# 10XGenomics/rust-pseudoaligner

Hardware: AMD Instinct MI355X
Metric: reads/sec pseudoaligned (whole node) on synthetic 150bp reads (higher is better)
Workload: dtype u64; 1 GPU; config3: ~202k-transcript synthetic GENCODE-scale index (K=24), error-free 150bp reads; read_len=150, k=24, transcripts=201914, kmers=103866252, index_bytes=7185579820

## Files before the change

### rust-pseudoaligner_amd/csrc/count_sort.hip

```cpp
#include <hip/hip_runtime.h>

#include <algorithm>

#include "kernels.hpp"
#include "pa_common.hpp"

namespace pa {
namespace {

constexpr uint32_t NO_KEY = 0xFFFFFFFFu;
#ifndef PA_MAX_BINS
#define PA_MAX_BINS 256
#endif
constexpr uint32_t MAX_BINS = PA_MAX_BINS;
constexpr uint64_t PA_COUNT_DIRECT_MAX_READS = 1u << 16;
constexpr uint32_t BIN_SLOTS = 1u << PA_KEY_BIN_SHIFT;
constexpr uint32_t CS_BLOCK = 1024;

struct KeyTops {
    const unsigned long long* top;
    uint64_t cap;
    const unsigned long long* extra_top;
    uint64_t extra_cap;
};
__device__ __forceinline__ uint64_t stream_len(const KeyTops k, uint64_t unused = 0) {
    (void)unused;
    unsigned long long t = *k.top, x = k.extra_top ? *k.extra_top : 0ull;
    if (t > k.cap) t = k.cap;
    if (x > k.extra_cap) x = k.extra_cap;
    return t + x;
}

constexpr uint32_t PT_BLOCK = 512, PT_PER = 16, PT_TILE = PT_BLOCK * PT_PER;

__device__ __forceinline__ uint64_t main_len(const KeyTops k) { const unsigned long long t = *k.top; return t < k.cap ? t : k.cap; }
__device__ __forceinline__ uint64_t extra_len(const KeyTops k) {
    const unsigned long long x = k.extra_top ? *k.extra_top : 0ull;
    return x < k.extra_cap ? x : k.extra_cap;
}
__device__ __forceinline__ uint32_t tiles_of(uint64_t n) { return (uint32_t)((n + PT_TILE - 1) / PT_TILE); }

__global__ __launch_bounds__(PT_BLOCK) void pa_keys_part_kernel(const uint32_t* __restrict__ keys, const KeyTops keys_top, uint32_t pass, uint32_t nbins,
                                                                uint32_t tcap, uint16_t* __restrict__ sorted, uint32_t* __restrict__ run_off) {
    __shared__ uint32_t cnt[MAX_BINS], lbase[MAX_BINS + 1];
    __shared__ __attribute__((aligned(16))) uint16_t stage[PT_TILE];
    const uint64_t m = main_len(keys_top);
    const uint64_t seg0 = pass ? m : 0, len = pass ? extra_len(keys_top) : m;
    const uint32_t tile0 = pass ? tiles_of(m) : 0u, ntiles = tiles_of(len);
    for (uint32_t t = blockIdx.x; t < ntiles; t += gridDim.x) {
        for (uint32_t b = threadIdx.x; b < nbins; b += PT_BLOCK) cnt[b] = 0;
        __syncthreads();
        const uint64_t t0 = (uint64_t)t * PT_TILE;
        uint32_t k[PT_PER], pos[PT_PER];
        const uint4* src = reinterpret_cast<const uint4*>(keys + seg0 + t0) + threadIdx.x;
#pragma unroll
        for (uint32_t j = 0; j < PT_PER / 4; ++j) {
            const uint64_t i = t0 + 4ull * (j * PT_BLOCK + threadIdx.x);
            const uint4 v = i < len ? src[j * PT_BLOCK] : uint4{NO_KEY, NO_KEY, NO_KEY, NO_KEY};
            k[4 * j] = v.x; k[4 * j + 1] = v.y; k[4 * j + 2] = v.z; k[4 * j + 3] = v.w;
        }
#pragma unroll
        for (uint32_t j = 0; j < PT_PER; ++j) pos[j] = k[j] != NO_KEY ? atomicAdd(&cnt[k[j] >> PA_KEY_BIN_SHIFT], 1u) : 0u;
        __syncthreads();
        for (uint32_t b = threadIdx.x; b <= nbins; b += PT_BLOCK) {
            uint32_t s = 0;
            for (uint32_t j = 0; j < b; ++j) s += cnt[j];
            lbase[b] = s;
            run_off[(uint64_t)b * tcap + tile0 + t] = s;
        }
        __syncthreads();
#pragma unroll
        for (uint32_t j = 0; j < PT_PER; ++j)
            if (k[j] != NO_KEY) stage[lbase[k[j] >> PA_KEY_BIN_SHIFT] + pos[j]] = (uint16_t)(k[j] & (BIN_SLOTS - 1));
        __syncthreads();
        uint4* dst = reinterpret_cast<uint4*>(sorted + (uint64_t)(tile0 + t) * PT_TILE);
        const uint32_t n8 = (lbase[nbins] + 7) / 8;
        for (uint32_t i = threadIdx.x; i < n8; i += PT_BLOCK) dst[i] = reinterpret_cast<const uint4*>(stage)[i];
        __syncthreads();
    }
}

constexpr uint32_t CG_LANES = 16, CG_DEPTH = 8;
__global__ __launch_bounds__(CS_BLOCK) void pa_keys_count_kernel(const uint16_t* __restrict__ src, const uint32_t* __restrict__ run_off, uint32_t tcap,
                                                                 const KeyTops keys_top, uint32_t parts, unsigned long long* __restrict__ counts,
                                                                 uint64_t counts_len) {
    extern __shared__ uint32_t tab[];
    const uint32_t bin = blockIdx.x / parts, part = blockIdx.x % parts;
    const uint64_t slot0 = (uint64_t)bin << PA_KEY_BIN_SHIFT;
    const uint32_t nslots = (uint32_t)(counts_len - slot0 < BIN_SLOTS ? counts_len - slot0 : BIN_SLOTS);
    for (uint32_t i = threadIdx.x; i < nslots; i += CS_BLOCK) tab[i] = 0;
    __syncthreads();
    const uint32_t ntiles = tiles_of(main_len(keys_top)) + tiles_of(extra_len(keys_top));
    const uint32_t ta = (uint32_t)((uint64_t)ntiles * part / parts), tb = (uint32_t)((uint64_t)ntiles * (part + 1) / parts);
    const uint32_t gl = threadIdx.x % CG_LANES, group = threadIdx.x / CG_LANES;
    const uint4* q = reinterpret_cast<const uint4*>(src);
    for (uint32_t t = ta + group; t < tb; t += CS_BLOCK / CG_LANES) {
        const uint64_t base = (uint64_t)t * PT_TILE;
        const uint64_t a = base + run_off[(uint64_t)bin * tcap + t], b = base + run_off[(uint64_t)(bin + 1) * tcap + t];
        const uint64_t a8 = (a + 7) & ~7ull, b8 = b & ~7ull;
        if (a8 >= b8) {
            for (uint64_t i = a + gl; i < b; i += CG_LANES) atomicAdd(&tab[src[i]], 1u);
            continue;
        }
        const uint32_t head = a + gl < a8 ? src[a + gl] : 0xFFFFu, tail = b8 + gl < b ? src[b8 + gl] : 0xFFFFu;
        for (uint64_t o0 = a8 / 8; o0 < b8 / 8; o0 += (uint64_t)CG_DEPTH * CG_LANES) {
            uint4 v[CG_DEPTH];
            bool in[CG_DEPTH];
#pragma unroll
            for (uint32_t j = 0; j < CG_DEPTH; ++j) {
                const uint64_t o = o0 + (uint64_t)j * CG_LANES + gl;
                in[j] = o < b8 / 8;
                v[j] = in[j] ? q[o] : uint4{0u, 0u, 0u, 0u};
            }
#pragma unroll
            for (uint32_t j = 0; j < CG_DEPTH; ++j)
                if (in[j]) {
                    atomicAdd(&tab[v[j].x & 0xFFFFu], 1u); atomicAdd(&tab[v[j].x >> 16], 1u);
                    atomicAdd(&tab[v[j].y & 0xFFFFu], 1u); atomicAdd(&tab[v[j].y >> 16], 1u);
                    atomicAdd(&tab[v[j].z & 0xFFFFu], 1u); atomicAdd(&tab[v[j].z >> 16], 1u);
                    atomicAdd(&tab[v[j].w & 0xFFFFu], 1u); atomicAdd(&tab[v[j].w >> 16], 1u);
                }
        }
        if (head != 0xFFFFu) atomicAdd(&tab[head], 1u);
        if (tail != 0xFFFFu) atomicAdd(&tab[tail], 1u);
    }
    __syncthreads();
    for (uint32_t i = threadIdx.x; i < nslots; i += CS_BLOCK) {
        const uint32_t c = tab[i];
        if (c) atomicAdd(counts + slot0 + i, (unsigned long long)c);
    }
}

__global__ __launch_bounds__(CS_BLOCK) void pa_keys_count_raw_kernel(const uint32_t* __restrict__ src, const KeyTops keys_top, unsigned long long* __restrict__ counts,
                                                                     uint64_t counts_len) {
    extern __shared__ uint32_t tab[];
    for (uint32_t i = threadIdx.x; i < counts_len; i += CS_BLOCK) tab[i] = 0;
    __syncthreads();
    const uint64_t n4 = stream_len(keys_top) / 4;
    const uint64_t a = n4 * blockIdx.x / gridDim.x, b = n4 * (blockIdx.x + 1) / gridDim.x;
    const uint4* q = reinterpret_cast<const uint4*>(src);
    for (uint64_t i = a + threadIdx.x; i < b; i += CS_BLOCK) {
        const uint4 v = q[i];
        if (v.x != NO_KEY) atomicAdd(&tab[v.x], 1u);
        if (v.y != NO_KEY) atomicAdd(&tab[v.y], 1u);
        if (v.z != NO_KEY) atomicAdd(&tab[v.z], 1u);
        if (v.w != NO_KEY) atomicAdd(&tab[v.w], 1u);
    }
    __syncthreads();
    for (uint32_t i = threadIdx.x; i < counts_len; i += CS_BLOCK) {
        const uint32_t c = tab[i];
        if (c) atomicAdd(counts + i, (unsigned long long)c);
    }
}

__global__ __launch_bounds__(256) void pa_keys_count_direct_kernel(const uint32_t* __restrict__ keys, const KeyTops keys_top, unsigned long long* __restrict__ counts) {
    const uint64_t n = stream_len(keys_top);
    for (uint64_t i = (uint64_t)blockIdx.x * blockDim.x + threadIdx.x; i < n; i += (uint64_t)gridDim.x * blockDim.x) {
        const uint32_t k = keys[i];
        if (k != NO_KEY) atomicAdd(counts + k, 1ull);
    }
}


}
uint64_t key_stream_capacity(uint64_t n_reads, uint32_t nwaves) {
    return (n_reads / PA_KEY_CHUNK + nwaves + 2) * PA_KEY_CHUNK;
}

static uint64_t nbins_of(uint64_t counts_len) { return (counts_len + BIN_SLOTS - 1) >> PA_KEY_BIN_SHIFT; }

static bool count_direct(uint64_t nbins, uint64_t n_reads) { return nbins > MAX_BINS || (nbins > 1 && n_reads <= PA_COUNT_DIRECT_MAX_READS); }

bool count_keys_partitioned(uint64_t counts_len, uint64_t n_reads) {
    const uint64_t nbins = nbins_of(counts_len);
    return nbins > 1 && !count_direct(nbins, n_reads);
}

static uint32_t tile_capacity(uint64_t keys_cap, uint64_t extra_cap) {
    return (uint32_t)((keys_cap + PT_TILE - 1) / PT_TILE + (extra_cap + PT_TILE - 1) / PT_TILE);
}

void count_keys_scratch(uint64_t counts_len, uint64_t n_reads, uint64_t keys_cap, uint64_t extra_cap, size_t* sorted_bytes, size_t* ctl_bytes) {
    *sorted_bytes = *ctl_bytes = 0;
    if (!count_keys_partitioned(counts_len, n_reads)) return;
    const uint64_t tcap = tile_capacity(keys_cap, extra_cap);
    *sorted_bytes = tcap * PT_TILE * sizeof(uint16_t);
    *ctl_bytes = (nbins_of(counts_len) + 1) * tcap * sizeof(uint32_t);
}

int launch_count_keys(const uint32_t* keys, const unsigned long long* keys_top_ptr, uint64_t keys_cap, const unsigned long long* extra_top, uint64_t extra_cap,
                      uint32_t* sorted, uint32_t* ctl, unsigned long long* counts, uint64_t counts_len, int num_cus, hipStream_t stream, uint64_t n_reads,
                      uint32_t pass) {
    if (counts_len == 0) return 0;
    const KeyTops keys_top{keys_top_ptr, keys_cap, extra_top, extra_cap};
    const uint64_t nbins = nbins_of(counts_len);
    const uint32_t cus = num_cus > 0 ? (uint32_t)num_cus : 256u;
    const bool partitioned = count_keys_partitioned(counts_len, n_reads);
    if (pass == 0) {
        if (!partitioned) return 0;
        const uint32_t tcap = tile_capacity(keys_cap, extra_cap);
        const uint32_t G = std::max<uint32_t>(1u, std::min<uint32_t>(cus * 4, (uint32_t)((keys_cap + PT_TILE - 1) / PT_TILE)));
        hipLaunchKernelGGL(pa_keys_part_kernel, dim3(G), dim3(PT_BLOCK), 0, stream, keys, keys_top, 0u, (uint32_t)nbins, tcap, reinterpret_cast<uint16_t*>(sorted), ctl);
        return (int)hipGetLastError();
    }
    const size_t lds = (size_t)(counts_len < BIN_SLOTS ? counts_len : BIN_SLOTS) * 4;
    if (lds > 48 * 1024) {
        hipError_t e = hipFuncSetAttribute(reinterpret_cast<const void*>(&pa_keys_count_kernel), hipFuncAttributeMaxDynamicSharedMemorySize, (int)lds);
        if (e == hipSuccess) e = hipFuncSetAttribute(reinterpret_cast<const void*>(&pa_keys_count_raw_kernel), hipFuncAttributeMaxDynamicSharedMemorySize, (int)lds);
        if (e != hipSuccess) return (int)e;
    }
    if (count_direct(nbins, n_reads)) {
        const uint32_t blocks = (uint32_t)std::min<uint64_t>((uint64_t)cus * 8, (keys_cap + extra_cap + 255) / 256 + 1);
        hipLaunchKernelGGL(pa_keys_count_direct_kernel, dim3(blocks), dim3(256), 0, stream, keys, keys_top, counts);
        return (int)hipGetLastError();
    }
    if (nbins == 1) {
        hipLaunchKernelGGL(pa_keys_count_raw_kernel, dim3(cus), dim3(CS_BLOCK), lds, stream, keys, keys_top, counts, counts_len);
        return (int)hipGetLastError();
    }
    const uint32_t tcap = tile_capacity(keys_cap, extra_cap);
    const uint32_t G1 = std::max<uint32_t>(1u, std::min<uint32_t>(cus * 4, (uint32_t)((extra_cap + PT_TILE - 1) / PT_TILE)));
    hipLaunchKernelGGL(pa_keys_part_kernel, dim3(G1), dim3(PT_BLOCK), 0, stream, keys, keys_top, 1u, (uint32_t)nbins, tcap, reinterpret_cast<uint16_t*>(sorted), ctl);
    uint32_t parts = std::max<uint32_t>(1u, (uint32_t)(cus / nbins));
    parts = std::max<uint32_t>(1u, (uint32_t)knob_int("PA_COUNT_PARTS", (int)parts));
    hipLaunchKernelGGL(pa_keys_count_kernel, dim3((uint32_t)nbins * parts), dim3(CS_BLOCK), lds, stream, reinterpret_cast<const uint16_t*>(sorted), (const uint32_t*)ctl, tcap,
                       keys_top, parts, counts, counts_len);
    return (int)hipGetLastError();
}

}
```

### rust-pseudoaligner_amd/csrc/device_index.hip

```cpp
#include <hip/hip_runtime.h>

#include <algorithm>
#include <cstdlib>
#include <cstring>
#include <thread>

#include "device_flatten.hpp"
#include "device_index.hpp"
#include "lane_steps.hpp"

using namespace pa;

namespace {

uint64_t list_hash_host(const uint32_t* v, uint32_t n) {
    uint64_t h = 0x243f6a8885a308d3ull ^ n;
    for (uint32_t i = 0; i < n; ++i) h = mix64(h ^ v[i]) + 0x9e3779b97f4a7c15ull;
    return h;
}

}

namespace pa {

void LaunchCtx::release() {
    if (side) (void)hipStreamSynchronize(side);
    ctl.release();
    for (DeviceBuffer<uint32_t>* b : {&spill, &trace, &novel, &keys, &keys_sorted, &keys_ctl, &defer}) b->release();
    for (hipEvent_t e : {ev0, ev1, ev2, ev3, fork, join})
        if (e) (void)hipEventDestroy(e);
    ev0 = ev1 = ev2 = ev3 = fork = join = nullptr;
    if (side) (void)hipStreamDestroy(side);
    side = nullptr;
    timed = false;
}

void* Parked::take(std::mutex& mu) {
    std::lock_guard<std::mutex> g(mu);
    if (held.empty()) return nullptr;
    void* obj = held.back().first;
    held.pop_back();
    return obj;
}
void Parked::put(std::mutex& mu, void* obj, void (*free_fn)(void*)) {
    {
        std::lock_guard<std::mutex> g(mu);
        if (held.size() < cap) {
            held.emplace_back(obj, free_fn);
            return;
        }
    }
    free_fn(obj);
}

void index_host_classes(const pa_index* idx, const uint32_t** ec, const uint32_t** class_ref, int* device) {
    *ec = idx->h_ec.data();
    *class_ref = idx->h_class_ref.data();
    *device = idx->device;
}
void index_pair_view(pa_index* idx, PairIndexView* out) {
    std::lock_guard<std::mutex> g(idx->mu);
    *out = PairIndexView{idx->dv, idx->d_class_table.get(), idx->class_table_size, idx->ovf, idx->device, idx->num_cus};
}
void index_host_class_text(pa_index* idx, const uint64_t** off, const char** text) {
    std::call_once(idx->class_text_once, [idx] {
        const uint32_t nc = idx->stats.num_classes;
        const uint32_t* ec = idx->h_ec.data();
        const uint32_t* cref = idx->h_class_ref.data();
        auto digits = [](uint32_t v) { uint32_t d = 1; while (v >= 10) { v /= 10; ++d; } return d; };
        std::vector<uint64_t>& off_v = idx->h_class_text_off;
        off_v.assign((size_t)nc + 1, 0);
        const int T = std::max(1, std::min(16, usable_threads()));
        const uint32_t* clen = idx->h_class_len.data();
        auto ids_of = [&](uint32_t c, const uint32_t*& ids, uint32_t& n) {
            ids = ec + 4ull * cref[c] + 1;
            n = clen[c];
        };
        {
            std::vector<std::thread> th;
            for (int t = 0; t < T; ++t)
                th.emplace_back([&, t] {
                    for (uint64_t c = (uint64_t)nc * t / T; c < (uint64_t)nc * (t + 1) / T; ++c) {
                        const uint32_t* ids; uint32_t n;
                        ids_of((uint32_t)c, ids, n);
                        uint64_t len = n ? 2ull * (n - 1) : 0;
                        for (uint32_t j = 0; j < n; ++j) len += digits(ids[j]);
                        off_v[c + 1] = len;
                    }
                });
            for (auto& x : th) x.join();
        }
        for (uint32_t c = 0; c < nc; ++c) off_v[c + 1] += off_v[c];
        idx->h_class_text.resize(off_v[nc] + 16);
        {
            std::vector<std::thread> th;
            for (int t = 0; t < T; ++t)
                th.emplace_back([&, t] {
                    for (uint64_t c = (uint64_t)nc * t / T; c < (uint64_t)nc * (t + 1) / T; ++c) {
                        const uint32_t* ids; uint32_t n;
                        ids_of((uint32_t)c, ids, n);
                        char* o = idx->h_class_text.data() + off_v[c];
                        for (uint32_t j = 0; j < n; ++j) {
                            if (j) { *o++ = ','; *o++ = ' '; }
                            char b[10]; int k = 10; uint32_t v = ids[j];
                            do { b[--k] = (char)('0' + v % 10); v /= 10; } while (v);
                            memcpy(o, b + k, (size_t)(10 - k)); o += 10 - k;
                        }
                    }
                });
            for (auto& x : th) x.join();
        }
    });
    *off = idx->h_class_text_off.data();
    *text = idx->h_class_text.data();
}
int index_device_class_text(pa_index* idx, const uint64_t** d_off, const uint8_t** d_text) {
    const uint64_t* off = nullptr;
    const char* txt = nullptr;
    index_host_class_text(idx, &off, &txt);
    std::lock_guard<std::mutex> g(idx->mu);
    if (!idx->d_class_text.get()) {
        if (hipSetDevice(idx->device) != hipSuccess) return fail(PA_ERR_HIP, "hipSetDevice failed");
        int e = upload(idx->d_class_text_off, off, idx->h_class_text_off.size());
        if (e == PA_OK) e = upload(idx->d_class_text, reinterpret_cast<const uint8_t*>(txt), idx->h_class_text.size());
        if (e != PA_OK) return e;
    }
    *d_off = idx->d_class_text_off.get();
    *d_text = idx->d_class_text.get();
    return PA_OK;
}
void* index_take_ingest_cache(pa_index* idx) { return idx->ingest_caches.take(idx->mu); }
void index_put_ingest_cache(pa_index* idx, void* cache, void (*free_fn)(void*)) { idx->ingest_caches.put(idx->mu, cache, free_fn); }
void* index_take_host_pipe(pa_index* idx) { return idx->host_pipes.take(idx->mu); }
void index_put_host_pipe(pa_index* idx, void* pipe, void (*free_fn)(void*)) { idx->host_pipes.put(idx->mu, pipe, free_fn); }

}

extern "C" {

void pa_index_destroy(pa_index* idx) {
    if (!idx) return;
    (void)hipSetDevice(idx->device);
    {
        std::vector<std::pair<void*, void (*)(void*)>> parked;
        { std::lock_guard<std::mutex> g(idx->mu); parked.swap(idx->ingest_caches.held); parked.insert(parked.end(), idx->host_pipes.held.begin(), idx->host_pipes.held.end()); idx->host_pipes.held.clear(); }
        for (auto& c : parked) c.second(c.first);
    }
    for (auto& kv : idx->ctxs) kv.second->release();
    delete idx;
}

int pa_index_create(const pa_flat_index* flat, int device, pa_index** out) {
    if (!flat || !out) return fail(PA_ERR_INVALID_ARG, "null argument");
    int rc = use_device(device);
    if (rc != PA_OK) return rc;
    FlatDevice fd;
    int threads = usable_threads();
    if (threads < 1) threads = 1;
    rc = flatten_for_device(*flat, threads, fd, true);
    if (rc != PA_OK) return rc;

    std::vector<uint32_t> ctab((size_t)fd.num_classes * 2 + 16, 0xFFFFFFFFu);
    for (uint32_t c = 0; c < fd.num_classes; ++c) {
        uint64_t j = list_hash_host(fd.ec.data() + 4ull * fd.class_ref[c] + 1, fd.class_len[c]) % ctab.size();
        while (ctab[j] != 0xFFFFFFFFu)
            if (++j == ctab.size()) j = 0;
        ctab[j] = c;
    }

    pa_index* idx = new (std::nothrow) pa_index();
    if (!idx) return fail(PA_ERR_OOM, "out of memory");
    idx->device = device;
    hipDeviceProp_t prop;
    if (hipGetDeviceProperties(&prop, device) == hipSuccess) idx->num_cus = prop.multiProcessorCount;
    if (idx->num_cus <= 0) idx->num_cus = 256;
    rc = upload(idx->d_blobs, fd.blobs);
    if (rc == PA_OK) rc = upload(idx->d_ledge, fd.ledge);
    if (rc == PA_OK) rc = device_fill_index(fd, idx->d_blobs.get(), idx->d_table, &fd.nbuckets);
    if (rc == PA_OK) rc = upload(idx->d_seg_g, fd.seg_g);
    if (rc == PA_OK) rc = upload(idx->d_seg_nid, fd.seg_nid);
    if (rc == PA_OK) rc = upload(idx->d_ec, fd.ec);
    if (rc == PA_OK) rc = upload(idx->d_class_ref, fd.class_ref);
    if (rc == PA_OK) rc = upload(idx->d_class_len, fd.class_len);
    if (rc == PA_OK) rc = upload(idx->d_class_table, ctab);
    if (rc == PA_OK) rc = upload(idx->d_wtable, fd.wtable);
    if (rc != PA_OK) { pa_index_destroy(idx); return rc; }
    idx->class_table_size = ctab.size();
    idx->dv = fd.host_view();
    idx->dv.table = idx->d_table.get();
    idx->dv.blobs = idx->d_blobs.get();
    idx->dv.ledge = idx->d_ledge.get();
    idx->dv.seg_g = idx->d_seg_g.get();
    idx->dv.seg_nid = idx->d_seg_nid.get();
    idx->h_ec = fd.ec;
    idx->h_class_ref = fd.class_ref;
    idx->h_class_len = fd.class_len;
    idx->dv.ec = idx->d_ec.get();
    idx->dv.class_ref = idx->d_class_ref.get();
    idx->dv.class_len = idx->d_class_len.get();
    idx->dv.wtable = idx->d_wtable.get();
    idx->dv.stream_nt = (fd.k <= 32 && fd.nbuckets * BUCKET_WORDS * 4 > (512ull << 20)) ? 1u : 0u;
    pa_index_stats& s = idx->stats;
    s.num_kmers = fd.num_kmers;
    s.table_slots = fd.nbuckets * SLOTS_PER_BUCKET;
    s.bytes_table = fd.nbuckets * BUCKET_WORDS * 4;
    s.bytes_graph = fd.blobs.size() + fd.ledge.size() * 4 + fd.seg_g.size() * 12;
    s.bytes_classes = (fd.ec.size() + fd.class_ref.size() + fd.class_len.size() + ctab.size() + fd.wtable.size()) * 4;
    s.bytes_total = s.bytes_table + s.bytes_graph + s.bytes_classes;
    s.num_nodes = fd.num_nodes;
    s.num_classes = fd.num_classes;
    s.k = fd.k;
    s.max_class_len = fd.max_class_len;
    *out = idx;
    return PA_OK;
}

int pa_index_create_multi(const pa_flat_index* flat, const int* devices, int ndev, pa_index** out) {
    if (!flat || !devices || !out || ndev < 1) return fail(PA_ERR_INVALID_ARG, "null argument or ndev < 1");
    for (int i = 0; i < ndev; ++i) out[i] = nullptr;
    for (int i = 0; i < ndev; ++i) {
        for (int j = 0; j < i; ++j)
            if (devices[j] == devices[i]) {
                for (int t = 0; t < i; ++t) { pa_index_destroy(out[t]); out[t] = nullptr; }
                return fail(PA_ERR_INVALID_ARG, "device %d listed twice", devices[i]);
            }
        const int rc = pa_index_create(flat, devices[i], &out[i]);
        if (rc != PA_OK) {
            const std::string why = last_error_ref();
            for (int t = 0; t <= i; ++t) { pa_index_destroy(out[t]); out[t] = nullptr; }
            return fail(rc, "device %d: %s", devices[i], why.c_str());
        }
    }
    return PA_OK;
}

int pa_index_get_stats(const pa_index* idx, pa_index_stats* stats) {
    if (!idx || !stats) return fail(PA_ERR_INVALID_ARG, "null argument");
    *stats = idx->stats;
    return PA_OK;
}

uint32_t pa_words_per_read(uint32_t max_read_len) { return (max_read_len + 31) / 32 ? (max_read_len + 31) / 32 : 1; }
size_t pa_tiles_words(uint64_t n_reads, uint32_t words_per_read) { return (size_t)((n_reads + 63) / 64) * words_per_read * 64; }

int pa_encode_reads_device(const pa_index* idx, const uint8_t* d_ascii, const uint64_t* d_offsets, uint64_t n_reads,
                           uint32_t words_per_read, uint64_t* d_tiles, uint32_t* d_lens, void* stream) {
    if (!idx || !d_ascii || !d_offsets || !d_tiles || !d_lens || words_per_read == 0) return fail(PA_ERR_INVALID_ARG, "null argument");
    PA_HIP_TRY(hipSetDevice(idx->device));
    const int e = launch_encode(d_ascii, d_offsets, n_reads, words_per_read, d_tiles, d_lens, static_cast<hipStream_t>(stream));
    if (e) return fail(PA_ERR_HIP, "encode launch: %s", hipGetErrorString((hipError_t)e));
    return PA_OK;
}

}

namespace pa {

static int env_int(const char* name, int dflt) { return knob_int(name, dflt); }

uint32_t spill_cap_of(uint32_t wpr) { return 256 * wpr + 24; }

static int pool_geometry(pa_index* idx, uint64_t n_reads, uint32_t wpr, uint32_t* grid, size_t* lds, uint32_t* slots) {
    const size_t cu_lds = 160 * 1024 - 4096;
    int per_cu = env_int("PA_MAP_BLOCKS_PER_CU", 3);
    uint32_t S = 0;
    for (; per_cu >= 1; --per_cu) {
        const size_t per_wave = cu_lds / (size_t)per_cu / (PA_MAP_BLOCK / 64);
        const size_t per_slot = pool_slot_bytes(wpr);
        if (per_wave < pool_fixed_bytes() + 64 * per_slot + 16) continue;
        S = (uint32_t)((per_wave - pool_fixed_bytes() - 16) / per_slot);
        break;
    }
    if (S < 64) return fail(PA_ERR_UNSUPPORTED, "reads of %u words do not fit the LDS of a compute unit", wpr);
    if (S > pool_max_slots()) S = pool_max_slots();
    const int want = env_int("PA_POOL_SLOTS", 0);
    if (want >= 64 && (uint32_t)want <= S) S = (uint32_t)want;
    *slots = S;
    *lds = pool_lds_bytes(wpr, S);
    int occ = 0;
    if (pool_kernel_occupancy(*lds, &occ) == 0 && occ >= 1 && occ < per_cu) per_cu = occ;
    const uint64_t ntiles = (n_reads + 63) / 64;
    const uint64_t waves_wanted = (ntiles + 7) / 8;
    uint64_t blocks = (waves_wanted + PA_MAP_BLOCK / 64 - 1) / (PA_MAP_BLOCK / 64);
    const uint64_t cap = (uint64_t)idx->num_cus * per_cu;
    if (blocks > cap) blocks = cap;
    if (blocks < 1) blocks = 1;
    *grid = (uint32_t)blocks;
    return PA_OK;
}

static int ctx_of(pa_index* idx, hipStream_t stream, std::shared_ptr<LaunchCtx>* out) {
    std::lock_guard<std::mutex> g(idx->mu);
    auto it = idx->ctxs.find(stream);
    if (it == idx->ctxs.end()) {
        std::shared_ptr<LaunchCtx> c(new (std::nothrow) LaunchCtx());
        if (!c) return fail(PA_ERR_OOM, "out of memory");
        const int rc = grow(c->ctl, 2);
        if (rc != PA_OK) return rc;
        it = idx->ctxs.emplace(stream, std::move(c)).first;
    }
    *out = it->second;
    return PA_OK;
}

int StreamCtx::open(pa_index* idx, hipStream_t stream) {
    PA_HIP_TRY(hipSetDevice(idx->device));
    const int rc = ctx_of(idx, stream, &cx);
    if (rc != PA_OK) return rc;
    lock = std::unique_lock<std::mutex>(cx->mu);
    return PA_OK;
}

int map_launch_locked(pa_index* idx, LaunchCtx* cx, hipStream_t stream, const MapLaunch& m) {
    const uint64_t n_reads = m.n_reads;
    const uint32_t wpr = m.wpr;
    MapCtl* const ctl = cx->ctl.get();
    if (n_reads >= 0xFFFFFFFFull) return fail(PA_ERR_UNSUPPORTED, "at most 2^32-2 reads per batch");
    if (wpr == 0 || wpr > (PA_MAX_READ_LEN + 31) / 32) return fail(PA_ERR_UNSUPPORTED, "words_per_read %u outside [1,%u]", wpr, (PA_MAX_READ_LEN + 31) / 32);
    uint32_t grid = 0;
    size_t lds = 0;
    uint32_t slots = 64;
    int rc = pool_geometry(idx, n_reads, wpr, &grid, &lds, &slots);
    if (rc != PA_OK) return rc;
    const uint32_t spill_cap = spill_cap_of(wpr);
    {
        const size_t per_block = (size_t)(PA_MAP_BLOCK / 64) * slots * spill_cap * 4 * (m.nodes ? 2 : 1);
        const size_t budget = (size_t)6 << 30;
        if ((size_t)grid * per_block > budget) grid = (uint32_t)std::max<size_t>(1, budget / per_block);
    }
    const size_t lanes = (size_t)grid * (PA_MAP_BLOCK / 64) * slots;
    rc = grow(cx->spill, lanes * spill_cap);
    if (rc != PA_OK) return rc;
    if (m.nodes) { rc = grow(cx->trace, lanes * spill_cap); if (rc != PA_OK) return rc; }
    PA_HIP_TRY(hipMemsetAsync(ctl, 0, sizeof(MapCtl), stream));
    MapParams p{};
    p.ix = idx->dv;
    p.tiles = m.tiles;
    p.lens = m.lens;
    p.uniform_len = m.uniform_len;
    p.n_reads = n_reads;
    p.wpr = wpr;
    p.allowed = m.allowed;
    p.results = m.results;
    p.arena = m.arena;
    p.arena_cap = m.arena_cap > PA_MAX_ARENA_ENTRIES ? PA_MAX_ARENA_ENTRIES : m.arena_cap;
    p.colour_out = m.colour;
    p.arena_top = &ctl->arena_top;
    p.status = &ctl->status;
    p.tile_ctr = &ctl->tile_ctr;
    p.spill = cx->spill.get();
    p.spill_cap = spill_cap;
    const uint64_t counts_len = (uint64_t)idx->stats.num_classes + 3;
    const uint64_t defer_cap = defer_capacity(n_reads, grid * (PA_MAP_BLOCK / 64));
    if ((rc = grow(cx->defer, defer_cap * 8))) return rc;
    p.defer = cx->defer.get();
    p.defer_top = &ctl->defer_top;
    p.defer_cap = defer_cap;
    p.keys_cap = 0;
    uint64_t keys_cap = 0;
    if (m.counts) {
        keys_cap = key_stream_capacity(n_reads, grid * (PA_MAP_BLOCK / 64));
        size_t sorted_bytes = 0, ctl_bytes = 0;
        count_keys_scratch(counts_len, n_reads, keys_cap, defer_cap, &sorted_bytes, &ctl_bytes);
        if ((rc = grow(cx->keys, keys_cap + defer_cap)) || (rc = grow(cx->keys_sorted, (sorted_bytes + 3) / 4)) || (rc = grow(cx->keys_ctl, (ctl_bytes + 3) / 4))) return rc;
        p.keys = cx->keys.get();
        p.keys_top = &ctl->keys_top;
        p.keys_cap = keys_cap;
        p.counts = reinterpret_cast<unsigned long long*>(m.counts);
    }
    p.class_table = idx->d_class_table.get();
    p.class_table_size = idx->class_table_size;
    p.pool_slots = slots;
    p.dbg = env_int("PA_MAP_STATS", 0) ? ctl->stats : nullptr;
    p.ablate = (uint32_t)env_int("PA_MAP_ABLATE", 0);
    pa_overflow* ovf = nullptr;
    { std::lock_guard<std::mutex> g(idx->mu); ovf = idx->ovf; }
    if (m.counts && ovf) {
        const uint64_t want = n_reads + 64;
        rc = grow(cx->novel, want * 2);
        if (rc != PA_OK) return rc;
        p.novel_list = cx->novel.get();
        p.novel_ctr = &ctl->novel_ctr;
        p.novel_cap = want;
        overflow_launch_params(ovf, p);
    }
    p.trace = m.nodes ? cx->trace.get() : nullptr;
    p.nodes_out = m.nodes;
    p.nodes_len = m.nodes_len;
    cx->last_grid = grid;
    cx->last_arena_cap = p.arena_cap;
    cx->timed = false;
    if (n_reads == 0) return PA_OK;
    bool timing = false;
    { std::lock_guard<std::mutex> g(idx->mu); timing = idx->timing; }
    if (timing) {
        if (!cx->ev0) { PA_HIP_TRY(hipEventCreate(&cx->ev0)); PA_HIP_TRY(hipEventCreate(&cx->ev1)); PA_HIP_TRY(hipEventCreate(&cx->ev2)); PA_HIP_TRY(hipEventCreate(&cx->ev3)); }
        PA_HIP_TRY(hipEventRecord(cx->ev0, stream));
    }
    const int e = launch_map_pool(p, grid, lds, stream);
    if (e) return fail(PA_ERR_HIP, "map launch (grid %u, lds %zu): %s", grid, lds, hipGetErrorString((hipError_t)e));
    if (timing) { PA_HIP_TRY(hipEventRecord(cx->ev1, stream)); cx->timed = true; }
    const bool overlap = m.counts && count_keys_partitioned(counts_len, n_reads);
    hipStream_t rs = stream;
    if (overlap) {
        if (!cx->side) {
            PA_HIP_TRY(hipStreamCreateWithFlags(&cx->side, hipStreamNonBlocking));
            PA_HIP_TRY(hipEventCreateWithFlags(&cx->fork, hipEventDisableTiming));
            PA_HIP_TRY(hipEventCreateWithFlags(&cx->join, hipEventDisableTiming));
        }
        PA_HIP_TRY(hipEventRecord(cx->fork, stream));
        PA_HIP_TRY(hipStreamWaitEvent(cx->side, cx->fork, 0));
        rs = cx->side;
    }
    {
        const int e1 = launch_resolve(p, defer_cap, keys_cap, idx->num_cus, rs);
        if (e1) return fail(PA_ERR_HIP, "resolve launch: %s", hipGetErrorString((hipError_t)e1));
    }
    if (timing) PA_HIP_TRY(hipEventRecord(cx->ev2, rs));
    if (overlap) {
        PA_HIP_TRY(hipEventRecord(cx->join, rs));
        const int e2 = launch_count_keys(p.keys, p.keys_top, keys_cap, p.defer_top, defer_cap, cx->keys_sorted.get(), cx->keys_ctl.get(), p.counts, counts_len,
                                         idx->num_cus, stream, n_reads, 0);
        if (e2) return fail(PA_ERR_HIP, "count launch: %s", hipGetErrorString((hipError_t)e2));
        PA_HIP_TRY(hipStreamWaitEvent(stream, cx->join, 0));
    }
    if (m.counts) {
        const int e2 = launch_count_keys(p.keys, p.keys_top, keys_cap, p.defer_top, defer_cap, cx->keys_sorted.get(), cx->keys_ctl.get(), p.counts, counts_len,
                                         idx->num_cus, stream, n_reads, 1);
        if (e2) return fail(PA_ERR_HIP, "count launch: %s", hipGetErrorString((hipError_t)e2));
        if (ovf) {
            rc = overflow_after_map(ovf, p.novel_list, p.novel_ctr, p.novel_cap, m.arena, stream);
            if (rc != PA_OK) return rc;
        }
    }
    if (timing) PA_HIP_TRY(hipEventRecord(cx->ev3, stream));
    return PA_OK;
}

int map_finish_locked(LaunchCtx* cx, hipStream_t stream, uint64_t* arena_used, uint64_t* arena_needed) {
    MapCtl ctl{};
    PA_HIP_TRY(hipMemcpyAsync(&ctl, cx->ctl.get(), offsetof(MapCtl, stats), hipMemcpyDeviceToHost, stream));
    PA_HIP_TRY(hipStreamSynchronize(stream));
    if (env_int("PA_MAP_STATS", 0)) {
        PA_HIP_TRY(hipMemcpy(&ctl, cx->ctl.get(), sizeof ctl, hipMemcpyDeviceToHost));
        static const char* names[] = {"refill", "seek", "fwd", "left", "pick+pop", "store+push", "fin_light", "fin_scan", "fin_coop", "fin_bits", "fin_mask", "fwd+seek", "fwd:issue", "fwd:wait", "fwd:wait+compute"};
        static_assert(sizeof names / sizeof names[0] == ST_NSTAT, "one name per statistics entry");
        const unsigned long long* d = ctl.stats;
        fprintf(stderr, "[pa map stats] grid=%u", cx->last_grid);
        for (uint32_t i = 0; i < ST_NSTAT; ++i)
            if (d[i])
                fprintf(stderr, " %s: %llu iters x %.1f lanes, %.0f ticks/iter;", names[i], d[i], (double)d[ST_NSTAT + i] / (double)d[i],
                        (double)d[2 * ST_NSTAT + i] / (double)d[i]);
        fprintf(stderr, " key stream %llu entries, deferred stream %llu entries\n", ctl.keys_top, ctl.defer_top);
    }
    const unsigned long long top = ctl.arena_top;
    if (arena_used) *arena_used = top < cx->last_arena_cap ? top : cx->last_arena_cap;
    if (arena_needed) *arena_needed = top;
    if (ctl.status & PA_STATUS_SPILL_OVERFLOW) return fail(PA_ERR_INTERNAL, "a per-launch stream (class rows, count keys or deferred reads) overflowed its buffer (should be impossible)");
    if (ctl.status & PA_STATUS_ARENA_FULL) return fail(PA_ERR_ARENA_FULL, "class arena too small: %llu entries needed", top);
    return PA_OK;
}

}

static int map_launch(pa_index* idx, void* stream, const MapLaunch& m) {
    StreamCtx s;
    const int rc = s.open(idx, static_cast<hipStream_t>(stream));
    if (rc != PA_OK) return rc;
    return map_launch_locked(idx, s.cx.get(), static_cast<hipStream_t>(stream), m);
}

static int timed_ctx(pa_index* idx, void* stream, const void* ms, StreamCtx* s) {
    if (!idx || !ms) return fail(PA_ERR_INVALID_ARG, "null argument");
    const int rc = s->open(idx, static_cast<hipStream_t>(stream));
    if (rc != PA_OK) return rc;
    if (!s->cx->timed) return fail(PA_ERR_INVALID_ARG, "no timed launch on this stream (pa_index_set_timing before the launch)");
    return PA_OK;
}

extern "C" {

int pa_index_release_stream(pa_index* idx, void* stream) {
    if (!idx) return fail(PA_ERR_INVALID_ARG, "null argument");
    std::shared_ptr<LaunchCtx> cx;
    {
        std::lock_guard<std::mutex> g(idx->mu);
        auto it = idx->ctxs.find(static_cast<hipStream_t>(stream));
        if (it == idx->ctxs.end()) return PA_OK;
        cx = std::move(it->second);
        idx->ctxs.erase(it);
    }
    std::lock_guard<std::mutex> g(cx->mu);
    hipError_t e = hipSetDevice(idx->device);
    if (e == hipSuccess) e = hipStreamSynchronize(static_cast<hipStream_t>(stream));
    cx->release();
    if (e != hipSuccess) return fail(PA_ERR_HIP, "pa_index_release_stream: %s", hipGetErrorString(e));
    return PA_OK;
}

int pa_map_batch_device(pa_index* idx, const uint64_t* d_tiles, const uint32_t* d_lens, uint64_t n_reads, uint32_t words_per_read,
                        uint32_t allowed_mismatches, pa_read_result* d_results, uint32_t* d_arena, uint64_t arena_cap,
                        uint32_t* d_colour, void* stream) {
    if (!idx || (n_reads && (!d_tiles || !d_lens || !d_results || !d_arena))) return fail(PA_ERR_INVALID_ARG, "null argument");
    MapLaunch m;
    m.tiles = d_tiles; m.lens = d_lens; m.n_reads = n_reads; m.wpr = words_per_read; m.allowed = allowed_mismatches;
    m.results = d_results; m.arena = d_arena; m.arena_cap = arena_cap; m.colour = d_colour;
    return map_launch(idx, stream, m);
}

int pa_map_count_batch_device(pa_index* idx, const uint64_t* d_tiles, const uint32_t* d_lens, uint64_t n_reads, uint32_t words_per_read,
                              uint32_t allowed_mismatches, pa_read_result* d_results, uint32_t* d_arena, uint64_t arena_cap,
                              uint64_t* d_counts, void* stream) {
    if (!idx || !d_counts || (n_reads && (!d_tiles || !d_lens || !d_results || !d_arena))) return fail(PA_ERR_INVALID_ARG, "null argument");
    MapLaunch m;
    m.tiles = d_tiles; m.lens = d_lens; m.n_reads = n_reads; m.wpr = words_per_read; m.allowed = allowed_mismatches;
    m.results = d_results; m.arena = d_arena; m.arena_cap = arena_cap; m.counts = d_counts;
    return map_launch(idx, stream, m);
}

int pa_map_count_batch_uniform_device(pa_index* idx, const uint64_t* d_tiles, uint32_t read_len, uint64_t n_reads, uint32_t words_per_read,
                                      uint32_t allowed_mismatches, pa_read_result* d_results, uint32_t* d_arena, uint64_t arena_cap, uint64_t* d_counts,
                                      void* stream) {
    if (!idx || !d_counts || (n_reads && (!d_tiles || !d_results || !d_arena))) return fail(PA_ERR_INVALID_ARG, "null argument");
    if (read_len == 0 || read_len > PA_MAX_READ_LEN || read_len > 32ull * words_per_read)
        return fail(PA_ERR_INVALID_ARG, "read_len %u does not fit %u words per read (or exceeds %u bases)", read_len, words_per_read, PA_MAX_READ_LEN);
    MapLaunch m;
    m.tiles = d_tiles; m.uniform_len = read_len; m.n_reads = n_reads; m.wpr = words_per_read; m.allowed = allowed_mismatches;
    m.results = d_results; m.arena = d_arena; m.arena_cap = arena_cap; m.counts = d_counts;
    return map_launch(idx, stream, m);
}

int pa_map_finish(pa_index* idx, void* stream, uint64_t* arena_used, uint64_t* arena_needed) {
    if (!idx) return fail(PA_ERR_INVALID_ARG, "null argument");
    StreamCtx s;
    const int rc = s.open(idx, static_cast<hipStream_t>(stream));
    if (rc != PA_OK) return rc;
    return map_finish_locked(s.cx.get(), static_cast<hipStream_t>(stream), arena_used, arena_needed);
}

int pa_index_set_timing(pa_index* idx, int on) {
    if (!idx) return fail(PA_ERR_INVALID_ARG, "null argument");
    std::lock_guard<std::mutex> g(idx->mu);
    idx->timing = on != 0;
    return PA_OK;
}

int pa_map_kernel_ms(pa_index* idx, void* stream, float* ms) {
    StreamCtx s;
    const int rc = timed_ctx(idx, stream, ms, &s);
    if (rc != PA_OK) return rc;
    PA_HIP_TRY(hipEventSynchronize(s.cx->ev1));
    PA_HIP_TRY(hipEventElapsedTime(ms, s.cx->ev0, s.cx->ev1));
    return PA_OK;
}

int pa_map_stage_ms(pa_index* idx, void* stream, float ms[3]) {
    StreamCtx s;
    const int rc = timed_ctx(idx, stream, ms, &s);
    if (rc != PA_OK) return rc;
    PA_HIP_TRY(hipEventSynchronize(s.cx->ev3));
    PA_HIP_TRY(hipEventElapsedTime(&ms[0], s.cx->ev0, s.cx->ev1));
    PA_HIP_TRY(hipEventElapsedTime(&ms[1], s.cx->ev1, s.cx->ev2));
    PA_HIP_TRY(hipEventElapsedTime(&ms[2], s.cx->ev2, s.cx->ev3));
    return PA_OK;
}

uint64_t pa_map_arena_hint(const pa_index* idx, uint64_t n_reads) {
    const uint64_t waves = idx ? (uint64_t)idx->num_cus * 8 * (PA_MAP_BLOCK / 64) : 8192;
    return n_reads * 8 + waves * PA_ARENA_CHUNK + 4096;
}

int pa_counts_by_barcode_device(pa_index* idx, const pa_read_result* d_results, const uint32_t* d_arena, const uint32_t* d_barcode, uint64_t n_reads,
                                uint32_t barcode_bits, uint64_t* d_keys, uint32_t* d_vals, uint64_t* n_entries, void* stream) {
    if (!idx || !n_entries || (n_reads && (!d_results || !d_arena || !d_barcode || !d_keys || !d_vals))) return fail(PA_ERR_INVALID_ARG, "null argument");
    PA_HIP_TRY(hipSetDevice(idx->device));
    return barcode_counts(idx->dv, idx->d_class_table.get(), idx->class_table_size, d_results, d_arena, d_barcode, n_reads,
                          barcode_bits, d_keys, d_vals, n_entries, static_cast<hipStream_t>(stream));
}

int pa_index_set_overflow(pa_index* idx, pa_overflow* ovf) {
    if (!idx) return fail(PA_ERR_INVALID_ARG, "null argument");
    if (ovf && overflow_device(ovf) != idx->device) return fail(PA_ERR_INVALID_ARG, "overflow table lives on device %d, the index on device %d", overflow_device(ovf), idx->device);
    std::lock_guard<std::mutex> g(idx->mu);
    idx->ovf = ovf;
    return PA_OK;
}

uint64_t pa_counts_len(const pa_index* idx) { return idx ? (uint64_t)idx->stats.num_classes + 3 : 0; }

int pa_counts_accumulate_device(pa_index* idx, const pa_read_result* d_results, const uint32_t* d_arena, const uint32_t* d_colour,
                                uint64_t n_reads, uint64_t* d_counts, void* stream) {
    if (!idx || !d_results || !d_arena || !d_counts) return fail(PA_ERR_INVALID_ARG, "null argument");
    PA_HIP_TRY(hipSetDevice(idx->device));
    const int e = launch_count(d_results, d_arena, d_colour, n_reads, idx->dv, idx->d_class_table.get(),
                               idx->class_table_size, reinterpret_cast<unsigned long long*>(d_counts), static_cast<hipStream_t>(stream));
    if (e) return fail(PA_ERR_HIP, "count launch: %s", hipGetErrorString((hipError_t)e));
    return PA_OK;
}

}
```

Before: 13.33 billion reads/s.

## Split key counting into per-pass partial tables with fold, overlap with resolve

Key counting in the partitioned path now runs per pass: pass 0 counts the main key stream right after map while resolve runs on the side stream, and pass 1 counts only the deferred extra keys after resolve. Each count block writes its LDS histogram to a partial buffer instead of issuing global 64-bit atomics, and a new fold kernel sums the partials per slot. The aim is to hide the main counting work behind resolve and to cut global atomic traffic. In exchange it adds scratch memory for the partials, an extra fold launch per pass, and a changed stream ordering.

```diff
diff --git a/rust-pseudoaligner_amd/csrc/count_sort.hip b/rust-pseudoaligner_amd/csrc/count_sort.hip
--- a/rust-pseudoaligner_amd/csrc/count_sort.hip
+++ b/rust-pseudoaligner_amd/csrc/count_sort.hip
@@ -1,6 +1,7 @@
 #include <hip/hip_runtime.h>
 
 #include <algorithm>
+#include <atomic>
 
 #include "kernels.hpp"
 #include "pa_common.hpp"
@@ -82,16 +83,16 @@
 
 constexpr uint32_t CG_LANES = 16, CG_DEPTH = 8;
 __global__ __launch_bounds__(CS_BLOCK) void pa_keys_count_kernel(const uint16_t* __restrict__ src, const uint32_t* __restrict__ run_off, uint32_t tcap,
-                                                                 const KeyTops keys_top, uint32_t parts, unsigned long long* __restrict__ counts,
-                                                                 uint64_t counts_len) {
-    extern __shared__ uint32_t tab[];
+                                                                 const KeyTops keys_top, uint32_t pass, uint32_t parts, uint32_t* __restrict__ partial) {
+    extern __shared__ __attribute__((aligned(16))) uint32_t tab[];
     const uint32_t bin = blockIdx.x / parts, part = blockIdx.x % parts;
-    const uint64_t slot0 = (uint64_t)bin << PA_KEY_BIN_SHIFT;
-    const uint32_t nslots = (uint32_t)(counts_len - slot0 < BIN_SLOTS ? counts_len - slot0 : BIN_SLOTS);
-    for (uint32_t i = threadIdx.x; i < nslots; i += CS_BLOCK) tab[i] = 0;
-    __syncthreads();
-    const uint32_t ntiles = tiles_of(main_len(keys_top)) + tiles_of(extra_len(keys_top));
-    const uint32_t ta = (uint32_t)((uint64_t)ntiles * part / parts), tb = (uint32_t)((uint64_t)ntiles * (part + 1) / parts);
+    const uint32_t tiles_main = tiles_of(main_len(keys_top));
+    const uint32_t tile0 = pass ? tiles_main : 0u, ntiles = pass ? tiles_of(extra_len(keys_top)) : tiles_main;
+    if (ntiles == 0) return;
+    uint4* const tab4 = reinterpret_cast<uint4*>(tab);
+    for (uint32_t i = threadIdx.x; i < BIN_SLOTS / 4; i += CS_BLOCK) tab4[i] = uint4{0u, 0u, 0u, 0u};
+    __syncthreads();
+    const uint32_t ta = tile0 + (uint32_t)((uint64_t)ntiles * part / parts), tb = tile0 + (uint32_t)((uint64_t)ntiles * (part + 1) / parts);
     const uint32_t gl = threadIdx.x % CG_LANES, group = threadIdx.x / CG_LANES;
     const uint4* q = reinterpret_cast<const uint4*>(src);
     for (uint32_t t = ta + group; t < tb; t += CS_BLOCK / CG_LANES) {
@@ -125,15 +126,30 @@
         if (tail != 0xFFFFu) atomicAdd(&tab[tail], 1u);
     }
     __syncthreads();
-    for (uint32_t i = threadIdx.x; i < nslots; i += CS_BLOCK) {
-        const uint32_t c = tab[i];
-        if (c) atomicAdd(counts + slot0 + i, (unsigned long long)c);
-    }
+    uint4* const dst = reinterpret_cast<uint4*>(partial + (uint64_t)blockIdx.x * BIN_SLOTS);
+    for (uint32_t i = threadIdx.x; i < BIN_SLOTS / 4; i += CS_BLOCK) dst[i] = tab4[i];
+}
+
+constexpr uint32_t FOLD_BLOCK = 256;
+__global__ __launch_bounds__(FOLD_BLOCK) void pa_keys_fold_kernel(const uint32_t* __restrict__ partial, const KeyTops keys_top, uint32_t pass, uint32_t parts,
+                                                                 unsigned long long* __restrict__ counts, uint64_t counts_len) {
+    if ((pass ? tiles_of(extra_len(keys_top)) : tiles_of(main_len(keys_top))) == 0) return;
+    const uint64_t s = (uint64_t)blockIdx.x * FOLD_BLOCK + threadIdx.x;
+    if (s >= counts_len) return;
+    const uint32_t* p = partial + (s >> PA_KEY_BIN_SHIFT) * parts * BIN_SLOTS + (s & (BIN_SLOTS - 1));
+    uint64_t sum = 0;
+    uint32_t j = 0;
+    for (; j + 4 <= parts; j += 4) {
+        const uint32_t a = p[(uint64_t)j * BIN_SLOTS], b = p[(uint64_t)(j + 1) * BIN_SLOTS], c = p[(uint64_t)(j + 2) * BIN_SLOTS], d = p[(uint64_t)(j + 3) * BIN_SLOTS];
+        sum += (uint64_t)a + b + c + d;
+    }
+    for (; j < parts; ++j) sum += p[(uint64_t)j * BIN_SLOTS];
+    if (sum) atomicAdd(counts + s, (unsigned long long)sum);
 }
 
 __global__ __launch_bounds__(CS_BLOCK) void pa_keys_count_raw_kernel(const uint32_t* __restrict__ src, const KeyTops keys_top, unsigned long long* __restrict__ counts,
                                                                      uint64_t counts_len) {
-    extern __shared__ uint32_t tab[];
+    extern __shared__ __attribute__((aligned(16))) uint32_t tab[];
     for (uint32_t i = threadIdx.x; i < counts_len; i += CS_BLOCK) tab[i] = 0;
     __syncthreads();
     const uint64_t n4 = stream_len(keys_top) / 4;
@@ -180,12 +196,53 @@
     return (uint32_t)((keys_cap + PT_TILE - 1) / PT_TILE + (extra_cap + PT_TILE - 1) / PT_TILE);
 }
 
+constexpr uint32_t COUNT_WGS_MAX = 256, COUNT_WGS_EXTRA = 64, COUNT_PARTS_EXTRA_MAX = 4;
+static uint32_t parts_cap(uint64_t nbins, uint32_t pass) {
+    if (pass == 0) return std::max<uint32_t>(1u, (uint32_t)(COUNT_WGS_MAX / nbins));
+    return std::min<uint32_t>(COUNT_PARTS_EXTRA_MAX, std::max<uint32_t>(1u, (uint32_t)(COUNT_WGS_EXTRA / nbins)));
+}
+static uint64_t run_off_words(uint64_t nbins, uint64_t tcap) { return ((nbins + 1) * tcap + 3) & ~3ull; }
+static uint64_t partial_words(uint64_t nbins, uint32_t pass) { return nbins * parts_cap(nbins, pass) * BIN_SLOTS; }
+
 void count_keys_scratch(uint64_t counts_len, uint64_t n_reads, uint64_t keys_cap, uint64_t extra_cap, size_t* sorted_bytes, size_t* ctl_bytes) {
     *sorted_bytes = *ctl_bytes = 0;
     if (!count_keys_partitioned(counts_len, n_reads)) return;
-    const uint64_t tcap = tile_capacity(keys_cap, extra_cap);
+    const uint64_t tcap = tile_capacity(keys_cap, extra_cap), nbins = nbins_of(counts_len);
     *sorted_bytes = tcap * PT_TILE * sizeof(uint16_t);
-    *ctl_bytes = (nbins_of(counts_len) + 1) * tcap * sizeof(uint32_t);
+    *ctl_bytes = (run_off_words(nbins, tcap) + partial_words(nbins, 0) + partial_words(nbins, 1)) * sizeof(uint32_t);
+}
+
+static hipError_t allow_large_lds() {
+    static std::atomic<uint64_t> done{0};
+    int dev = 0;
+    hipError_t e = hipGetDevice(&dev);
+    if (e != hipSuccess) return e;
+    const uint64_t bit = 1ull << (dev & 63);
+    if (dev < 64 && (done.load(std::memory_order_acquire) & bit)) return hipSuccess;
+    const int lds = (int)(BIN_SLOTS * sizeof(uint32_t));
+    e = hipFuncSetAttribute(reinterpret_cast<const void*>(&pa_keys_count_kernel), hipFuncAttributeMaxDynamicSharedMemorySize, lds);
+    if (e == hipSuccess) e = hipFuncSetAttribute(reinterpret_cast<const void*>(&pa_keys_count_raw_kernel), hipFuncAttributeMaxDynamicSharedMemorySize, lds);
+    if (e == hipSuccess && dev < 64) done.fetch_or(bit, std::memory_order_release);
+    return e;
+}
+
+static int launch_pass(const uint32_t* keys, const KeyTops keys_top, uint64_t seg_cap, uint32_t* sorted, uint32_t* ctl, unsigned long long* counts, uint64_t counts_len,
+                       uint32_t cus, hipStream_t stream, uint32_t pass) {
+    const uint64_t nbins = nbins_of(counts_len);
+    const uint32_t tcap = tile_capacity(keys_top.cap, keys_top.extra_cap);
+    const uint32_t G = std::max<uint32_t>(1u, std::min<uint32_t>(cus * 4, (uint32_t)((seg_cap + PT_TILE - 1) / PT_TILE)));
+    hipLaunchKernelGGL(pa_keys_part_kernel, dim3(G), dim3(PT_BLOCK), 0, stream, keys, keys_top, pass, (uint32_t)nbins, tcap, reinterpret_cast<uint16_t*>(sorted), ctl);
+    uint32_t parts = parts_cap(nbins, pass);
+    if (pass == 0) {
+        parts = std::max<uint32_t>(1u, std::min<uint32_t>(parts, (uint32_t)(cus / nbins)));
+        parts = std::min<uint32_t>(parts_cap(nbins, 0), std::max<uint32_t>(1u, (uint32_t)knob_int("PA_COUNT_PARTS", (int)parts)));
+    }
+    uint32_t* partial = ctl + run_off_words(nbins, tcap) + (pass ? partial_words(nbins, 0) : 0);
+    hipLaunchKernelGGL(pa_keys_count_kernel, dim3((uint32_t)nbins * parts), dim3(CS_BLOCK), BIN_SLOTS * sizeof(uint32_t), stream, reinterpret_cast<const uint16_t*>(sorted),
+                       (const uint32_t*)ctl, tcap, keys_top, pass, parts, partial);
+    hipLaunchKernelGGL(pa_keys_fold_kernel, dim3((uint32_t)((counts_len + FOLD_BLOCK - 1) / FOLD_BLOCK)), dim3(FOLD_BLOCK), 0, stream, (const uint32_t*)partial, keys_top, pass,
+                       parts, counts, counts_len);
+    return (int)hipGetLastError();
 }
 
 int launch_count_keys(const uint32_t* keys, const unsigned long long* keys_top_ptr, uint64_t keys_cap, const unsigned long long* extra_top, uint64_t extra_cap,
@@ -196,35 +253,20 @@
     const uint64_t nbins = nbins_of(counts_len);
     const uint32_t cus = num_cus > 0 ? (uint32_t)num_cus : 256u;
     const bool partitioned = count_keys_partitioned(counts_len, n_reads);
-    if (pass == 0) {
-        if (!partitioned) return 0;
-        const uint32_t tcap = tile_capacity(keys_cap, extra_cap);
-        const uint32_t G = std::max<uint32_t>(1u, std::min<uint32_t>(cus * 4, (uint32_t)((keys_cap + PT_TILE - 1) / PT_TILE)));
-        hipLaunchKernelGGL(pa_keys_part_kernel, dim3(G), dim3(PT_BLOCK), 0, stream, keys, keys_top, 0u, (uint32_t)nbins, tcap, reinterpret_cast<uint16_t*>(sorted), ctl);
-        return (int)hipGetLastError();
-    }
     const size_t lds = (size_t)(counts_len < BIN_SLOTS ? counts_len : BIN_SLOTS) * 4;
-    if (lds > 48 * 1024) {
-        hipError_t e = hipFuncSetAttribute(reinterpret_cast<const void*>(&pa_keys_count_kernel), hipFuncAttributeMaxDynamicSharedMemorySize, (int)lds);
-        if (e == hipSuccess) e = hipFuncSetAttribute(reinterpret_cast<const void*>(&pa_keys_count_raw_kernel), hipFuncAttributeMaxDynamicSharedMemorySize, (int)lds);
+    if (lds > 48 * 1024 && (partitioned || pass)) {
+        const hipError_t e = allow_large_lds();
         if (e != hipSuccess) return (int)e;
     }
+    if (partitioned)
+        return launch_pass(keys, keys_top, pass ? extra_cap : keys_cap, sorted, ctl, counts, counts_len, cus, stream, pass);
+    if (pass == 0) return 0;
     if (count_direct(nbins, n_reads)) {
         const uint32_t blocks = (uint32_t)std::min<uint64_t>((uint64_t)cus * 8, (keys_cap + extra_cap + 255) / 256 + 1);
         hipLaunchKernelGGL(pa_keys_count_direct_kernel, dim3(blocks), dim3(256), 0, stream, keys, keys_top, counts);
         return (int)hipGetLastError();
     }
-    if (nbins == 1) {
-        hipLaunchKernelGGL(pa_keys_count_raw_kernel, dim3(cus), dim3(CS_BLOCK), lds, stream, keys, keys_top, counts, counts_len);
-        return (int)hipGetLastError();
-    }
-    const uint32_t tcap = tile_capacity(keys_cap, extra_cap);
-    const uint32_t G1 = std::max<uint32_t>(1u, std::min<uint32_t>(cus * 4, (uint32_t)((extra_cap + PT_TILE - 1) / PT_TILE)));
-    hipLaunchKernelGGL(pa_keys_part_kernel, dim3(G1), dim3(PT_BLOCK), 0, stream, keys, keys_top, 1u, (uint32_t)nbins, tcap, reinterpret_cast<uint16_t*>(sorted), ctl);
-    uint32_t parts = std::max<uint32_t>(1u, (uint32_t)(cus / nbins));
-    parts = std::max<uint32_t>(1u, (uint32_t)knob_int("PA_COUNT_PARTS", (int)parts));
-    hipLaunchKernelGGL(pa_keys_count_kernel, dim3((uint32_t)nbins * parts), dim3(CS_BLOCK), lds, stream, reinterpret_cast<const uint16_t*>(sorted), (const uint32_t*)ctl, tcap,
-                       keys_top, parts, counts, counts_len);
+    hipLaunchKernelGGL(pa_keys_count_raw_kernel, dim3(cus), dim3(CS_BLOCK), lds, stream, keys, keys_top, counts, counts_len);
     return (int)hipGetLastError();
 }
 
diff --git a/rust-pseudoaligner_amd/csrc/device_index.hip b/rust-pseudoaligner_amd/csrc/device_index.hip
--- a/rust-pseudoaligner_amd/csrc/device_index.hip
+++ b/rust-pseudoaligner_amd/csrc/device_index.hip
@@ -411,23 +411,23 @@
         PA_HIP_TRY(hipEventRecord(cx->fork, stream));
         PA_HIP_TRY(hipStreamWaitEvent(cx->side, cx->fork, 0));
         rs = cx->side;
+        const int e2 = launch_count_keys(p.keys, p.keys_top, keys_cap, p.defer_top, defer_cap, cx->keys_sorted.get(), cx->keys_ctl.get(), p.counts, counts_len,
+                                         idx->num_cus, stream, n_reads, 0);
+        if (e2) return fail(PA_ERR_HIP, "count launch: %s", hipGetErrorString((hipError_t)e2));
     }
     {
         const int e1 = launch_resolve(p, defer_cap, keys_cap, idx->num_cus, rs);
         if (e1) return fail(PA_ERR_HIP, "resolve launch: %s", hipGetErrorString((hipError_t)e1));
     }
     if (timing) PA_HIP_TRY(hipEventRecord(cx->ev2, rs));
-    if (overlap) {
-        PA_HIP_TRY(hipEventRecord(cx->join, rs));
-        const int e2 = launch_count_keys(p.keys, p.keys_top, keys_cap, p.defer_top, defer_cap, cx->keys_sorted.get(), cx->keys_ctl.get(), p.counts, counts_len,
-                                         idx->num_cus, stream, n_reads, 0);
-        if (e2) return fail(PA_ERR_HIP, "count launch: %s", hipGetErrorString((hipError_t)e2));
-        PA_HIP_TRY(hipStreamWaitEvent(stream, cx->join, 0));
-    }
     if (m.counts) {
         const int e2 = launch_count_keys(p.keys, p.keys_top, keys_cap, p.defer_top, defer_cap, cx->keys_sorted.get(), cx->keys_ctl.get(), p.counts, counts_len,
-                                         idx->num_cus, stream, n_reads, 1);
+                                         idx->num_cus, rs, n_reads, 1);
         if (e2) return fail(PA_ERR_HIP, "count launch: %s", hipGetErrorString((hipError_t)e2));
+        if (overlap) {
+            PA_HIP_TRY(hipEventRecord(cx->join, rs));
+            PA_HIP_TRY(hipStreamWaitEvent(stream, cx->join, 0));
+        }
         if (ovf) {
             rc = overflow_after_map(ovf, p.novel_list, p.novel_ctr, p.novel_cap, m.arena, stream);
             if (rc != PA_OK) return rc;
```

Result: no change. 13.27 billion reads/s (-0.5%).
